# marl/l3embedding

Hardware: AMD Instinct MI355X
Metric: AVC training pairs/sec (1s audio + 224x224 frame) (higher is better)
Workload: dtype f32; 1 GPU; full cnn_L3_melspec2 AVC training step (audio+vision+fusion, fwd+bwd+Adam), batch 64 per GPU, global batch 64, fp32, inputs resident in HBM; global_batch=64, parallelism=dp1, fp32_conv=f4x4

## Files before the change

l3embedding_amd/csrc/conv_path.h:

```cpp
#pragma once
#include "kernels.h"

namespace l3 {

ConvGeom conv_geom(int n, int h, int w, int cin, int cout, int kh, int kw, bool same, int f2x2);
ConvGeom conv_dgrad_geom(const ConvGeom& g);

struct ConvStorage {
    bool mixed = false;
    bool x_bf16 = false, y_bf16 = false, dy_bf16 = false, dx_bf16 = false;
};

enum ConvFwd { CF_BF16_STORED, CF_BF16_CAST, CF_FIRST, CF_FP32 };
enum ConvWgrad { WG_BF16_STORED, WG_BF16_CAST, WG_FP32 };
enum ConvDgrad { DG_NONE, DG_SMALL, DG_BF16_STORED, DG_BF16_CAST, DG_WINO, DG_FLIPPED };
struct ConvFwdPath {
    ConvFwd path = CF_FP32;
    bool wino_filter = false;
    double executed = -1.0;
};
struct ConvWgradPath {
    ConvWgrad path = WG_FP32;
    double executed = -1.0;
};
struct ConvDgradPath {
    ConvDgrad path = DG_NONE;
    double executed = -1.0;
};
ConvFwdPath conv_resolve_fwd(const ConvGeom& g, const ConvStorage& st, bool have_u);
ConvWgradPath conv_resolve_wgrad(const ConvGeom& g, const ConvStorage& st);
ConvDgradPath conv_resolve_dgrad(const ConvGeom& g, const ConvGeom& dg, const ConvStorage& st, bool have_u);
int conv_fwd_stat_blocks(const ConvFwdPath& p, const ConvGeom& g);
int conv_dgrad_bn_blocks(const ConvDgradPath& p, const ConvGeom& dg, bool dx_bf16, bool bn_x_bf16);

struct ConvBufs {
    const float* x = nullptr;
    const float* w = nullptr;
    const float* bias = nullptr;
    float* y = nullptr;
    float* dx = nullptr;
    float* dw = nullptr;
    float* wprep = nullptr;
    float* wino_u = nullptr;
    bool u_ready = false;
    float* wg_part = nullptr;
    float* stat_part = nullptr;
    int stat_mode = 0;
    const BnBwdFuse* bn_bwd = nullptr;
};
void conv_run_fwd(const ConvFwdPath& p, const ConvGeom& g, const ConvStorage& st, const ConvBufs& b, hipStream_t s);
void conv_run_wgrad(const ConvWgradPath& p, const ConvGeom& g, const ConvBufs& b, hipStream_t s);
void conv_run_dgrad(const ConvDgradPath& p, const ConvGeom& g, const ConvGeom& dg, const ConvStorage& st, const ConvBufs& b, hipStream_t s);

}
```

l3embedding_amd/csrc/conv_path.hip:

```cpp
#include "conv_path.h"

namespace l3 {

ConvGeom conv_geom(int n, int h, int w, int cin, int cout, int kh, int kw, bool same, int f2x2) {
    ConvGeom g{n, h, w, cin, 0, 0, cout, kh, kw, 0, 0};
    if (same) {
        tf_same(h, kh, 1, &g.Ho, &g.padT);
        tf_same(w, kw, 1, &g.Wo, &g.padL);
    } else {
        g.Ho = h - kh + 1;
        g.Wo = w - kw + 1;
    }
    g.f2x2 = f2x2;
    return g;
}

ConvGeom conv_dgrad_geom(const ConvGeom& g) {
    ConvGeom dg{g.N, g.Ho, g.Wo, g.Cout, g.H, g.W, g.Cin, g.KH, g.KW, g.KH - 1 - g.padT, g.KW - 1 - g.padL};
    dg.f2x2 = g.f2x2;
    dg.solo = g.solo;
    return dg;
}

ConvFwdPath conv_resolve_fwd(const ConvGeom& g, const ConvStorage& st, bool have_u) {
    ConvFwdPath p;
    const bool mp = st.mixed && conv_bf16_ok(g);
    p.path = mp ? (st.x_bf16 ? CF_BF16_STORED : CF_BF16_CAST) : conv_first_ok(g) ? CF_FIRST : CF_FP32;
    p.wino_filter = have_u && !mp && conv_wino_ok(g);
    p.executed = p.wino_filter ? conv_wino_executed_flops(g) : -1.0;
    return p;
}

ConvWgradPath conv_resolve_wgrad(const ConvGeom& g, const ConvStorage& st) {
    ConvWgradPath p;
    const bool wbf = st.mixed && conv_wgrad_bf16_ok(g);
    p.path = !wbf ? WG_FP32 : st.x_bf16 && st.dy_bf16 ? WG_BF16_STORED : WG_BF16_CAST;
    p.executed = conv_wgrad_executed_flops(g, wbf);
    return p;
}

ConvDgradPath conv_resolve_dgrad(const ConvGeom& g, const ConvGeom& dg, const ConvStorage& st, bool have_u) {
    ConvDgradPath p;
    const bool dbf = st.mixed && conv_bf16_ok(dg), wino = have_u && conv_wino_ok(dg);
    p.path = conv_dgrad_small_ok(g) ? DG_SMALL : dbf ? (st.dy_bf16 ? DG_BF16_STORED : DG_BF16_CAST) : wino ? DG_WINO : DG_FLIPPED;
    p.executed = wino && !dbf ? conv_wino_executed_flops(dg) : -1.0;
    return p;
}

int conv_fwd_stat_blocks(const ConvFwdPath& p, const ConvGeom& g) {
    return p.path == CF_BF16_STORED ? conv_bf16_stat_blocks(g)
           : p.path == CF_FIRST     ? conv_first_stat_blocks(g)
           : p.path == CF_FP32 && p.wino_filter ? conv_wino_stat_blocks(g) : 0;
}

int conv_dgrad_bn_blocks(const ConvDgradPath& p, const ConvGeom& dg, bool dx_bf16, bool bn_x_bf16) {
    int blocks = -1;
    if (p.path == DG_BF16_STORED && dx_bf16 && bn_x_bf16 && conv_bf16_halo_ok(dg)) blocks = conv_bf16_stat_blocks(dg);
    if (p.path == DG_WINO && !dx_bf16 && !bn_x_bf16 && conv_wino_ok(dg)) blocks = conv_wino_stat_blocks(dg);
    return blocks;
}

void conv_run_fwd(const ConvFwdPath& p, const ConvGeom& g, const ConvStorage& st, const ConvBufs& b, hipStream_t s) {
    if (p.wino_filter && !b.u_ready) conv_wino_transform_weights(b.w, b.wino_u, g, false, s);
    switch (p.path) {
        case CF_BF16_STORED:
            conv_weights_bf16(b.w, b.wprep, g.KH, g.KW, g.Cin, g.Cout, true, s);
            conv_bf16_fwd(b.x, b.wprep, b.bias, b.y, g, s, true, b.stat_part, b.stat_mode, st.y_bf16);
            break;
        case CF_BF16_CAST:
            conv_flip_weights(b.w, b.wprep, g.KH, g.KW, g.Cin, g.Cout, s);
            conv_bf16_fwd(b.x, b.wprep, b.bias, b.y, g, s);
            break;
        case CF_FIRST:
            conv_first_fwd(b.x, b.w, b.bias, b.y, g, s, b.stat_part, b.stat_mode, st.y_bf16);
            break;
        case CF_FP32:
            conv_fwd(b.x, b.w, b.bias, b.y, g, s, p.wino_filter ? b.wino_u : nullptr, b.stat_part, b.stat_mode);
            break;
    }
}

void conv_run_wgrad(const ConvWgradPath& p, const ConvGeom& g, const ConvBufs& b, hipStream_t s) {
    conv_wgrad(b.x, b.y, b.dw, b.wg_part, g, s, p.path != WG_FP32, p.path == WG_BF16_STORED);
}

void conv_run_dgrad(const ConvDgradPath& p, const ConvGeom& g, const ConvGeom& dg, const ConvStorage& st, const ConvBufs& b, hipStream_t s) {
    switch (p.path) {
        case DG_SMALL:
            (void)conv_dgrad_small(b.y, b.w, b.dx, g, s);
            break;
        case DG_BF16_STORED:
            conv_weights_bf16(b.w, b.wprep, g.KH, g.KW, g.Cin, g.Cout, false, s);
            conv_bf16_fwd(b.y, b.wprep, nullptr, b.dx, dg, s, true, b.stat_part, 0, st.dx_bf16, b.bn_bwd);
            break;
        case DG_BF16_CAST:
            conv_bf16_fwd(b.y, b.w, nullptr, b.dx, dg, s);
            break;
        case DG_WINO:
            conv_wino_transform_weights(b.w, b.wino_u, dg, true, s);
            conv_fwd(b.y, nullptr, nullptr, b.dx, dg, s, b.wino_u, b.stat_part, 0, b.bn_bwd);
            break;
        case DG_FLIPPED:
            conv_flip_weights(b.w, b.wprep, g.KH, g.KW, g.Cin, g.Cout, s);
            conv_fwd(b.y, b.wprep, nullptr, b.dx, dg, s);
            break;
        case DG_NONE: break;
    }
}

}
```

l3embedding_amd/csrc/conv_wino4.hip:

```cpp
#include "kernels.h"
#include "device_common.h"

#include <stdlib.h>
#include <string.h>

#include <mutex>
#include <vector>

namespace l3 {

namespace {

struct Wino4Args {
    const float* x;
    const float* u;
    const float* bias;
    float* y;
    int N, H, W, Cin, Cout;
    int TY, TX;
    int tiles;
    int mblocks, nblocks, nchunks;
    float inv_tpi, inv_tx;
    float* stat_part;
    int stat_mode;
// ... 581 lines not shown
        if (t < 128) {
            const int c32 = t & 31, which = (t >> 5) & 1, jn = t >> 6;
            float sum = 0.f;
#pragma unroll
            for (int r = 0; r < NS; ++r) sum += red[((jn * 2 + which) * NS + r) * 32 + c32];
            a.stat_part[((size_t)mb * 2 + which) * a.Cout + n0 + jn * 32 + c32] = sum;
        }
    }
    if (!worker) __builtin_amdgcn_s_waitcnt(0x0070 | (0xF << 8));
    if (dyn && wave == 11 && lane0 == 0) {
        asm volatile("" ::: "memory");
        int nx = -1;
        if (has_next) {
            nx = wq_base(a.lt_first, xcd) + 8 * claim_k;
            if (nx >= a.lt_end) nx = wq_claim(a.work, xcd, 1, a.lt_first, a.lt_end);
        }
        Qw[it & 1] = nx;
    }
    have0 = has_next;
    }
    if (dyn && t == 0) wq_leave(a.work, (int)gridDim.x);
}

__global__ __launch_bounds__(256) void wino4_weights_kernel(const float* __restrict__ w, float* __restrict__ u, int Cin,
                                                            int Cout, int dgrad) {
    const int idx = blockIdx.x * 256 + threadIdx.x;
    if (idx >= Cin * Cout) return;
    const int k = idx % Cout, c = idx / Cout;
    float g[3][3];
#pragma unroll
    for (int kh = 0; kh < 3; ++kh)
#pragma unroll
        for (int kw = 0; kw < 3; ++kw)
            g[kh][kw] = dgrad ? w[((size_t)((2 - kh) * 3 + (2 - kw)) * Cout + k) * Cin + c]
                              : w[((size_t)(kh * 3 + kw) * Cin + c) * Cout + k];
    auto gmul = [](float a0, float a1, float a2, float* o) {
        const float s02 = a0 + a2;
        o[0] = a0;
        o[1] = (-1.f / 3.f) * (s02 + a1);
        o[2] = (1.f / 3.f) * (s02 - a1);
        o[3] = (1.f / 15.f) * fmaf(2.f, a1, fmaf(4.f, a2, a0));
        o[4] = (-4.f / 15.f) * fmaf(-2.f, a1, fmaf(4.f, a0, a2));
        o[5] = a2;
    };
    float gg[6][3];
#pragma unroll
    for (int kw = 0; kw < 3; ++kw) {
        float o[6];
        gmul(g[0][kw], g[1][kw], g[2][kw], o);
#pragma unroll
        for (int xi = 0; xi < 6; ++xi) gg[xi][kw] = o[xi];
    }
    const int c8 = c >> 3, hf = (c >> 2) & 1, sub = (c >> 1) & 1, c2 = c & 1;
#pragma unroll
    for (int xi = 0; xi < 6; ++xi) {
        float o[6];
        gmul(gg[xi][0], gg[xi][1], gg[xi][2], o);
#pragma unroll
        for (int nu = 0; nu < 6; ++nu)
            u[(((((size_t)(xi * 6 + nu) * (Cin >> 3) + c8) * 2 + sub) * 2 + hf) * Cout + k) * 2 + c2] = o[nu];
    }
}

template <int SM>
__global__ __launch_bounds__(256) void wino4_tail_reduce_kernel(Wino4Args a) {
    __shared__ float red[2][64][16];
    const int t = threadIdx.x, q = t & 3, slot = t >> 2;
    const int blk = (int)blockIdx.x >> 2, cg = (int)blockIdx.x & 3;
    const int lt = a.lt_first + blk;
    const int logical = xcd_remap(lt, a.mblocks * a.nblocks);
    const int nb = logical % a.nblocks, mb = logical / a.nblocks;
    const int n0 = nb * 64, T0 = mb * W4_TILES;
    const int cl = cg * 16 + 4 * q;
    const int ch = n0 + cl;
    f32x4 bz = {0.f, 0.f, 0.f, 0.f};
    if (a.bias != nullptr) bz = *reinterpret_cast<const f32x4*>(a.bias + ch);
    f32x4 bsc = bz, bsh = bz, bmu = bz, brs = bz;
    if constexpr (SM == 2) {
        bsc = *reinterpret_cast<const f32x4*>(a.bb.scale + ch);
        bsh = *reinterpret_cast<const f32x4*>(a.bb.shift + ch);
        bmu = *reinterpret_cast<const f32x4*>(a.bb.mean + ch);
        const f32x4 var = *reinterpret_cast<const f32x4*>(a.bb.var + ch);
#pragma unroll
        for (int c = 0; c < 4; ++c) brs[c] = rsqrtf(var[c] + a.bb.eps);
// ... 176 lines not shown
}

bool conv_wino4_selected(const ConvGeom& g) {
    const char* env = l3_knob("L3_WINO4");
    const int min_cin = env ? atoi(env) : 64;
    return !g.f2x2 && min_cin > 0 && g.Cin >= min_cin && g.Cin >= 16 && g.Cin % 8 == 0 && g.Cout % 64 == 0 &&
           (size_t)36 * g.Cin * g.Cout * 4 < (1ull << 31);
}

double conv_wino4_executed_flops(const ConvGeom& g) {
    return 2.0 * 36.0 * (double)g.N * ((g.H + 3) / 4) * ((g.W + 3) / 4) * (double)g.Cin * (double)g.Cout;
}

size_t conv_wino4_tail_scratch_bytes() { return (size_t)304 * W4_TILES * 16 * 64 * sizeof(float); }

int conv_wino4_blocks(const ConvGeom& g, int n) { return (n * ((g.H + 3) / 4) * ((g.W + 3) / 4) + W4_TILES - 1) / W4_TILES; }

void conv_wino4_transform_weights(const float* w, float* u, const ConvGeom& g, bool from_fwd_for_dgrad, hipStream_t s) {
    const int total = g.Cin * g.Cout;
    hipLaunchKernelGGL(wino4_weights_kernel, dim3((total + 255) / 256), dim3(256), 0, s, w, u, g.Cin, g.Cout,
                       from_fwd_for_dgrad ? 1 : 0);
}

void conv_wino4_launch(const float* x, const float* u, const float* bias, float* y, const ConvGeom& g, int n, hipStream_t s,
                       float* stat_part, int stat_mode, const BnBwdFuse* bn_bwd) {
    Wino4Args a;
    a.solo = g.solo;
    a.dynamic = g.dynamic;
    a.tail_buf = g.tail_scratch;
    a.tail_cap = g.tail_scratch_bytes;
    a.x = x; a.u = u; a.bias = bias; a.y = y;
    a.N = n; a.H = g.H; a.W = g.W; a.Cin = g.Cin; a.Cout = g.Cout;
    a.TY = (g.H + 3) / 4;
    a.TX = (g.W + 3) / 4;
    a.tiles = n * a.TY * a.TX;
    a.mblocks = conv_wino4_blocks(g, n);
    a.nblocks = g.Cout / 64;
    a.nchunks = g.Cin / 8;
    a.inv_tpi = 1.0f / (float)(a.TY * a.TX);
    a.inv_tx = 1.0f / (float)a.TX;
    a.stat_part = stat_part;
    a.stat_mode = stat_mode;
    a.bb = BnBwdFuse{nullptr, nullptr, nullptr, nullptr, nullptr, 0.f, 0};
    a.stagger_cycles = 0;
    a.stagger_groups = 1;
    a.lt_first = 0;
// ... 21 lines not shown
```

l3embedding_amd/csrc/engine.hip:

```cpp
#include <hip/hip_runtime.h>
#include "knobs.h"

#include <cmath>
#include <cstdio>
#include <cstdlib>
#include <cstring>
#include <map>
#include <string>
#include <vector>

#include "../../include/l3hip.h"
#include "comm.h"
#include "conv_path.h"
#include "featprep.h"
#include "kernels.h"

namespace {

using namespace l3;

static thread_local std::string g_create_error;

constexpr float BN_EPS = 1e-3f;
constexpr float BN_MOMENTUM = 0.99f;
// ... 18 lines not shown

struct Param {
    std::string name;
    int ndim = 0;
    int64_t shape[4] = {1, 1, 1, 1};
    bool trainable = false;
    int kind = 0;
    int64_t numel = 0;
    int bucket = 0;
    float* d = nullptr;
    float* g = nullptr;
};

enum FirstWgrad { FW_NONE, FW_AUG, FW_AUG_DEFERRED };
struct ConvPlan {
    ConvStorage st;
    ConvFwdPath fwd;
    int stat_mode = 0;
    FirstWgrad aug = FW_NONE;
    ConvWgradPath wgrad;
    bool colsum = false;
    ConvDgradPath dgrad;
    int bwd_bn = -1;
    double fwd_bytes = 0.0, wg_bytes = 0.0, dg_bytes = 0.0;
};
enum BnStats { BS_PARTIALS, BS_FAST, BS_PLAIN, BS_MOVING };
enum BnBwd { BB_BY_FIRST_CONV, BB_FAST_POOLED, BB_FAST, BB_FAST_DEFERRED, BB_PLAIN };
struct BnPlan {
    BnStats stats = BS_MOVING;
    int stat_blocks = 0;
    BnBwd bwd = BB_PLAIN;
    int bwd_blocks = 0;
    double fwd_bytes = 0.0, bwd_bytes = 0.0;
};

struct Op {
    OpKind kind;
    std::string name;
    int in = 0, out = 0;
    int block = 0, bucket = 0;
    int kh = 0, kw = 0, cout = 0;
    bool same = false;
    ConvGeom geom{};
    ConvGeom dgeom{};
    int p_kernel = -1, p_bias = -1;
    float* wflip = nullptr;
    float *wino_uf = nullptr, *wino_ud = nullptr;
    int in_bn = -1;
    bool fused_first = false;
    bool defer_apply = false;
    int bn_defer = -1;
    float *xaug = nullptr, *gaug = nullptr;
    ConvGeom ageom{};
    int bn_follow = -1;
    bool need_dx = true;
    int dy_to_bn = -1;
    float* xwin = nullptr;
    int p_gamma = -1, p_beta = -1, p_mmean = -1, p_mvar = -1;
    bool fused_relu = false;
    bool prerelu = false;
    int fuse_pool = -1;
    int bias_param = -1;
    bool fused_into_bn = false;
    bool bias_by_bn = false;
    float *mean = nullptr, *var = nullptr, *scale = nullptr, *shift = nullptr;
    float *biased_mean = nullptr, *biased_var = nullptr;
    PoolGeom pg{};
    ConvPlan cp{};
    BnPlan bp{};
};

struct Tower {
    std::string prefix;
    std::vector<Tensor> t;
    std::vector<Op> ops;
    int nblocks = 0;
    int emb_conv_op = -1;
    bool training = false;
};

struct FrontendDef {
    int n_dft, n_hop, same, n_mels, sqrt_out, db, loglambda;
    const char* layer_name;
};

struct ProfRec {
    int family;
    hipEvent_t a, b;
    double flops;
    double executed;
    double bytes;
    const char* tag;
};

}

struct l3_engine {
    l3_config cfg{};
    int B = 0;
    hipStream_t stream = nullptr;
    bool own_stream = false;
    hipStream_t side = nullptr;
    hipEvent_t ev_fork = nullptr, ev_join = nullptr;
    float *red_scratch2 = nullptr, *wg_scratch2 = nullptr;
    float *stat_scratch = nullptr, *stat_scratch2 = nullptr;
    size_t stat_max = 0;
    float* w4_tail = nullptr;
    bool overlap = true;
    BnMovingEntry* bn_table = nullptr;
    int bn_table_n = 0, bn_table_max_c = 0;
    std::string err;
    l3::DeviceBufs bufs;

    std::vector<Param> params;
    std::map<std::string, int> pindex;
    float *arena_p = nullptr, *arena_g = nullptr, *arena_m = nullptr, *arena_v = nullptr;
    int64_t n_train = 0;
    struct Segment { int64_t off, n; bool l2; };
    std::vector<Segment> segments;
    struct Bucket { int64_t off, n; };
    std::vector<Bucket> buckets;
    int64_t adam_t = 0;
    int64_t bn_step = 0;

    Tower vis, aud;
    FrontendDef fe{};
    FrontendCfg fcfg{};
    int p_real = -1, p_imag = -1, p_mel = -1;
    bool consts_dirty = true;
    float *wdft = nullptr, *melw = nullptr, *frames = nullptr, *spec = nullptr, *smax = nullptr;
    bool dft_consts_done = false;
    float *dft_win = nullptr, *dft_b1 = nullptr, *dft_b2 = nullptr, *dft_tw = nullptr, *dft_y = nullptr, *dft_a2 = nullptr, *dft_nyq = nullptr;
    int *mel_start = nullptr, *mel_len = nullptr, *mel_off = nullptr;
// ... 556 lines not shown
            memcpy(row, &real[(size_t)t * nb], nb * sizeof(float));
            memcpy(row + nb, &imag[(size_t)t * nb], nb * sizeof(float));
        }
        HIPCHK(e, hipMemcpy(e->wdft, w.data(), w.size() * 4, hipMemcpyHostToDevice));
    }
    if (f.n_mels) {
        std::vector<float> fb((size_t)nb * f.n_mels);
        HIPCHK(e, hipMemcpy(fb.data(), e->params[e->p_mel].d, fb.size() * 4, hipMemcpyDeviceToHost));
        MelBands bands;
        mel_pack_bands(fb.data(), nb, f.n_mels, bands);
        const std::vector<int>&st = bands.start, &ln = bands.len, &of = bands.off;
        const std::vector<float>& packed = bands.w;
        if ((int64_t)packed.size() > e->melw_cap) {
            e->err = "mel filterbank too dense for the band buffer";
            return L3_EINVAL;
        }
        HIPCHK(e, hipMemcpy(e->melw, packed.data(), packed.size() * 4, hipMemcpyHostToDevice));
        HIPCHK(e, hipMemcpy(e->mel_start, st.data(), st.size() * 4, hipMemcpyHostToDevice));
        HIPCHK(e, hipMemcpy(e->mel_len, ln.data(), ln.size() * 4, hipMemcpyHostToDevice));
        HIPCHK(e, hipMemcpy(e->mel_off, of.data(), of.size() * 4, hipMemcpyHostToDevice));
    }
    e->consts_dirty = false;
    return L3_OK;
}

int alloc_everything(l3_engine* e, uint64_t seed) {
    const int B = e->B;
    const int nbuckets = 1 + e->vis.nblocks + e->aud.nblocks;
    std::vector<int64_t> offs(e->params.size(), -1);
    int64_t off = 0;
    e->buckets.resize(nbuckets);
    for (int b = 0; b < nbuckets; ++b) {
        e->buckets[b].off = off;
        for (int pass = 0; pass < 2; ++pass) {
            const int64_t seg0 = off;
            for (size_t i = 0; i < e->params.size(); ++i) {
                Param& p = e->params[i];
                if (!p.trainable || p.bucket != b) continue;
                const bool is_l2 = p.kind == PK_KERNEL;
                if ((pass == 0) != is_l2) continue;
                offs[i] = off;
                off += (p.numel + 3) / 4 * 4;
            }
            if (off > seg0) e->segments.push_back({seg0, off - seg0, pass == 0});
        }
        e->buckets[b].n = off - e->buckets[b].off;
// ... 191 lines not shown
            }
        }
    }
    if (e->vis.ops.back().kind != OP_POOL || e->aud.ops.back().kind != OP_POOL) {
        e->err = "tower must end in a pooling layer";
        return L3_EINVAL;
    }
    if ((rc = dev_alloc_t(e, &e->red_scratch, red_max))) return rc;
    if ((rc = dev_alloc_t(e, &e->wg_scratch, wg_max))) return rc;
    if ((rc = dev_alloc_t(e, &e->sq_scratch, 2048))) return rc;
    if (stat_max && (rc = dev_alloc_t(e, &e->stat_scratch, stat_max))) return rc;
    {
        bool any_w4 = false;
        for (Tower* tw : {&e->vis, &e->aud})
            for (auto& op : tw->ops)
                if (op.kind == OP_CONV && (op.wino_uf || op.wino_ud)) any_w4 = true;
        if (any_w4 && e->cfg.dtype != L3_DTYPE_BF16 && (rc = dev_alloc_t(e, &e->w4_tail, conv_wino4_tail_scratch_bytes() / sizeof(float)))) return rc;
    }
    if (e->side) {
        if ((rc = dev_alloc_t(e, &e->red_scratch2, red_max))) return rc;
        if ((rc = dev_alloc_t(e, &e->wg_scratch2, wg_max))) return rc;
        if (stat_max && (rc = dev_alloc_t(e, &e->stat_scratch2, stat_max))) return rc;
    }
    return L3_OK;
}

int run_frontend(l3_engine* e) {
    int rc = rebuild_consts(e);
    if (rc) return rc;
    const FrontendCfg& f = e->fcfg;
    const int B = e->B;
    const int M = B * f.n_frames;
    const bool mag = e->cfg.frontend == L3_FRONTEND_MINISPEC && f.n_mels > 0;
    if (f.factored) {
        const int N1 = f.N1, N2 = f.N2;
        const int form = knob_int("L3_DFT_FACTORED", 1);
        if (form != 2 && f.n_mels > 0 && N1 == 32 && N2 == 64) {
            const double m1 = (double)M * N2, m2 = (double)M * N1;
            ProfScope ps(e, F_FRONTEND, 2.0 * M * (double)f.n_dft * 2.0 * f.n_freq + 2.0 * M * (double)f.n_freq * f.n_mels, nullptr,
                         2.0 * m1 * N1 * 2 * N1 + 2.0 * m2 * 2 * N2 * N2);
            dft_fused(e->audio, e->dft_win, e->dft_b1, e->dft_b2, e->dft_tw, e->melw, e->mel_start, e->mel_len, e->mel_off, e->aud.t[0].d, B,
                      AUDIO_T, f, e->stream, mag);
            if (f.db) db_normalize(e->aud.t[0].d, e->smax, B, e->aud.t[0].batch_stride, e->cfg.db_max_scope, e->stream);
            return L3_OK;
        }
        {
            ProfScope ps(e, F_FRONTEND, 0.0);
// ... 23 lines not shown
        {
            ProfScope ps(e, F_FRONTEND, 0.0);
            frame_audio(e->audio, e->frames, B, AUDIO_T, f, e->stream);
        }
        ConvGeom g{1, 1, M, f.n_dft, 1, M, f.ncols_pad, 1, 1, 0, 0};
        ProfScope ps(e, F_FRONTEND, 2.0 * M * (double)f.n_dft * 2.0 * f.n_freq);
        conv_fwd(e->frames, e->wdft, nullptr, e->spec, g, e->stream);
    }
    {
        ProfScope ps(e, F_FRONTEND, f.n_mels ? 2.0 * B * f.n_frames * (double)f.n_freq * f.n_mels : 0.0);
        spec_to_features(e->spec, e->melw, e->mel_start, e->mel_len, e->mel_off, e->aud.t[0].d, B, f, e->stream, e->dft_nyq, mag);
        if (f.db) db_normalize(e->aud.t[0].d, e->smax, B, e->aud.t[0].batch_stride, e->cfg.db_max_scope, e->stream);
    }
    return L3_OK;
}

static inline double act_bytes(const Tensor& t) { return (double)t.numel() * (t.d_bf16 ? 2.0 : 4.0); }
static inline double grad_bytes(const Tensor& t) { return (double)t.numel() * (t.g_bf16 ? 2.0 : 4.0); }

int plan_tower(l3_engine* e, Tower& tw, bool training, int solo) {
    static const int epi_stats = knob_int("L3_EPILOGUE_STATS", 1);
    const bool bf16 = e->cfg.dtype == L3_DTYPE_BF16;
    tw.training = training;
    auto fits = [&](const Op& cv, int blocks, int C) {
        if ((size_t)blocks * 2 * C <= e->stat_max) return true;
        e->err = cv.name + ": " + std::to_string(blocks) + " partial blocks of " + std::to_string(C) + " channels exceed the statistics scratch (" +
                 std::to_string(e->stat_max) + " floats)";
        return false;
    };
    auto defers = [&](const Op& bn) {
        return training && bn.defer_apply && bn.fuse_pool < 0 && bn_fast_ok(tw.t[bn.in].C) && tw.t[bn.in].d_bf16 == tw.t[bn.out].g_bf16;
    };
    for (auto& op : tw.ops) op.bp = BnPlan{};
    for (auto& op : tw.ops) {
        if (op.kind != OP_CONV) continue;
        op.geom.solo = op.dgeom.solo = solo;
        op.geom.dynamic = op.dgeom.dynamic = e->comm != nullptr ? 1 : 0;
        float* ts = solo ? e->w4_tail : nullptr;
        op.geom.tail_scratch = op.dgeom.tail_scratch = ts;
        op.geom.tail_scratch_bytes = op.dgeom.tail_scratch_bytes = ts ? conv_wino4_tail_scratch_bytes() : 0;

        const Tensor &x = tw.t[op.in], &y = tw.t[op.out];
        const double wbytes = (double)e->params[op.p_kernel].numel * 4.0;
        ConvPlan& p = op.cp = ConvPlan{};
        p.st = ConvStorage{bf16, x.d_bf16, y.d_bf16, y.g_bf16, x.g_bf16};
        p.fwd = conv_resolve_fwd(op.geom, p.st, op.wino_uf != nullptr);
        p.fwd_bytes = act_bytes(x) + act_bytes(y) + wbytes;
        const int nblk = conv_fwd_stat_blocks(p.fwd, op.geom);
        if (epi_stats && training && op.bn_follow >= 0 && e->stat_max > 0 && nblk > 0) {
            if (!fits(op, nblk, op.geom.Cout)) return L3_ESTATE;
            p.stat_mode = tw.ops[op.bn_follow].prerelu ? 2 : 1;
            tw.ops[op.bn_follow].bp.stat_blocks = nblk;
        }
        if (training && op.in_bn >= 0) {
            const Op* fb = op.bn_defer >= 0 && defers(tw.ops[op.bn_defer]) ? &tw.ops[op.bn_defer] : nullptr;
            p.aug = fb ? FW_AUG_DEFERRED : FW_AUG;
            p.wg_bytes = (double)x.rows() * op.ageom.Cin * 4.0 + (fb ? act_bytes(tw.t[fb->in]) + grad_bytes(tw.t[fb->out]) : grad_bytes(y));
            continue;
        }
        p.wgrad = conv_resolve_wgrad(op.geom, p.st);
        p.wg_bytes = act_bytes(x) + grad_bytes(y) + wbytes;
        p.colsum = !op.bias_by_bn;
        if (!op.need_dx) continue;
        p.dgrad = conv_resolve_dgrad(op.geom, op.dgeom, p.st, op.wino_ud != nullptr);
        p.dg_bytes = grad_bytes(y) + grad_bytes(x) + wbytes;
        Op* bn = training && op.dy_to_bn >= 0 && e->stat_max > 0 ? &tw.ops[op.dy_to_bn] : nullptr;
        if (bn != nullptr && bn->fuse_pool >= 0 && (bn->xwin == nullptr || x.batch_stride != (int64_t)x.H * x.W * x.C)) bn = nullptr;
        if (bn == nullptr) continue;
        const int blocks = conv_dgrad_bn_blocks(p.dgrad, op.dgeom, x.g_bf16, tw.t[bn->in].d_bf16);
        if (blocks < 0) continue;
        if (!fits(op, blocks, op.dgeom.Cout)) return L3_ESTATE;
        p.bwd_bn = op.dy_to_bn;
        bn->bp.bwd_blocks = blocks;
    }
    for (auto& op : tw.ops) {
        if (op.kind != OP_BN) continue;
        const Tensor &x = tw.t[op.in], &y = tw.t[op.out];
        const Tensor& out = op.fuse_pool >= 0 ? tw.t[tw.ops[op.fuse_pool].out] : y;
        BnPlan& p = op.bp;
        p.stats = !training ? BS_MOVING : p.stat_blocks > 0 ? BS_PARTIALS : op.prerelu || x.d_bf16 ? BS_FAST : BS_PLAIN;
        p.bwd = training && op.fused_first ? BB_BY_FIRST_CONV : !bn_fast_ok(x.C) ? BB_PLAIN : op.fuse_pool >= 0 ? BB_FAST_POOLED
                : defers(op) ? BB_FAST_DEFERRED : BB_FAST;
        p.fwd_bytes = (!training ? 0.0 : p.stat_blocks > 0 ? (double)p.stat_blocks * 2 * x.C * 4 : act_bytes(x)) + act_bytes(x) + act_bytes(out);
        if (p.bwd == BB_BY_FIRST_CONV) p.fwd_bytes += act_bytes(x) + (double)x.rows() * (&op + 1)->ageom.Cin * 4.0;
        if (op.fuse_pool >= 0 && training && op.xwin != nullptr) p.fwd_bytes += (double)out.numel() * (x.d_bf16 ? 2.0 : 4.0);
        p.bwd_bytes = p.bwd == BB_PLAIN ? 2.0 * (act_bytes(x) + grad_bytes(y)) + grad_bytes(x)
                                        : (p.bwd_blocks > 0 ? (double)p.bwd_blocks * 2 * x.C * 4 : act_bytes(x) + grad_bytes(out)) +
                                              (p.bwd == BB_FAST_DEFERRED ? 0.0 : act_bytes(x) + grad_bytes(out) + grad_bytes(x));
    }
    return L3_OK;
}

void tower_forward(l3_engine* e, Tower& tw) {
    const bool training = tw.training;
    for (auto& op : tw.ops) {
        Tensor& x = tw.t[op.in];
        Tensor& y = tw.t[op.out];
        switch (op.kind) {
            case OP_CONV: {
                const ConvPlan& p = op.cp;
                ConvBufs b;
                b.x = x.d, b.w = e->params[op.p_kernel].d, b.bias = e->params[op.p_bias].d, b.y = y.d;
                b.wprep = op.wflip, b.wino_u = op.wino_uf;
                b.stat_part = p.stat_mode ? e->stat_scratch : nullptr, b.stat_mode = p.stat_mode;
                ProfScope ps(e, F_CONV_FWD, conv_flops(op.geom), op.name.c_str(), p.fwd.executed);
                ps.bytes(p.fwd_bytes);
                conv_run_fwd(p.fwd, op.geom, p.st, b, e->stream);
                break;
            }
            case OP_BN: {
                const BnPlan& p = op.bp;
                ProfScope ps(e, F_ELEMWISE, 0.0);
                ps.bytes(p.fwd_bytes);
                const float* gamma = e->params[op.p_gamma].d;
                const float* beta = e->params[op.p_beta].d;
                switch (p.stats) {
                    case BS_PARTIALS:
                        bn_stats_from_partials(e->stat_scratch, p.stat_blocks, e->params[op.bias_param].d, gamma, beta, op.mean, op.var,
                                               op.scale, op.shift, x.rows(), x.C, BN_EPS, op.prerelu ? 1 : 0, e->stream);
                        break;
                    case BS_FAST:
                        bn_stats_fast(x.d, gamma, beta, op.mean, op.var, op.scale, op.shift, e->red_scratch, x.rows(), x.C, BN_EPS,
                                      op.prerelu ? 1 : 0, e->stream, x.d_bf16 ? 1 : 0);
                        break;
                    case BS_PLAIN:
                        bn_stats(x.d, gamma, beta, op.mean, op.var, op.scale, op.shift, e->red_scratch, x.rows(), x.C, BN_EPS, e->stream);
// ... 91 lines not shown
                if (p.aug != FW_NONE) {
                    ProfScope ps(e, F_CONV_WGRAD, conv_flops(op.geom), op.name.c_str());
                    ps.bytes(p.wg_bytes);
                    const Op& bn = tw.ops[op.in_bn];
                    if (p.aug == FW_AUG_DEFERRED) {
                        const Op& fb = tw.ops[op.bn_defer];
                        const Tensor &bi = tw.t[fb.in], &bo = tw.t[fb.out];
                        const float* co = bn_bwd_fast_coeffs(e->red_scratch, op.cout);
                        const FirstWgFuse f{bi.d, bo.g, fb.scale, fb.shift, co, co + op.cout, co + 2 * op.cout, fb.fused_relu ? 1 : 0,
                                            bi.d_bf16 ? 1 : 0};
                        conv_wgrad(op.xaug, nullptr, op.gaug, e->wg_scratch, op.ageom, e->stream, false, false, &f);
                    } else {
                        conv_wgrad(op.xaug, y.g, op.gaug, e->wg_scratch, op.ageom, e->stream);
                    }
                    first_conv_grads(op.gaug, w, e->params[bn.p_gamma].d, e->params[bn.p_beta].d, e->params[op.p_kernel].g,
                                     e->params[bn.p_gamma].g, e->params[bn.p_beta].g,
                                     op.bias_by_bn && p.aug == FW_AUG ? nullptr : e->params[op.p_bias].g, op.kh * op.kw, x.C, op.cout,
                                     e->stream);
                    break;
                }
                ConvBufs b;
                b.x = x.d, b.w = w, b.y = y.g, b.dx = x.g, b.dw = e->params[op.p_kernel].g;
                b.wprep = op.wflip, b.wino_u = op.wino_ud, b.wg_part = e->wg_scratch;
                {
                    ProfScope ps(e, F_CONV_WGRAD, conv_flops(op.geom), op.name.c_str(), p.wgrad.executed);
                    ps.bytes(p.wg_bytes);
                    conv_run_wgrad(p.wgrad, op.geom, b, e->stream);
                }
                if (p.colsum) {
                    ProfScope ps(e, F_ELEMWISE, 0.0);
                    ps.bytes(grad_bytes(y));
                    colsum(y.g, e->params[op.p_bias].g, e->red_scratch, y.rows(), y.C, e->stream);
                }
                if (p.dgrad.path == DG_NONE) break;
                ProfScope ps(e, F_CONV_DGRAD, conv_flops(op.geom), op.name.c_str(), p.dgrad.executed);
                ps.bytes(p.dg_bytes);
                BnBwdFuse bb{};
                if (p.bwd_bn >= 0) {
                    bb = bn_bwd_fuse(tw, tw.ops[p.bwd_bn]);
                    b.bn_bwd = &bb, b.stat_part = e->stat_scratch;
                }
                conv_run_dgrad(p.dgrad, op.geom, op.dgeom, p.st, b, e->stream);
                break;
            }
            default: break;
        }
// ... 107 lines not shown
    e->bn_table_n = (int)tab.size();
    e->bn_pack_floats = off;
    BnMovingEntry* dev = nullptr;
    if (int rc = dev_alloc_t(e, &dev, tab.size() + 1)) return rc;
    HIPCHK(e, hipMemcpy(dev, tab.data(), tab.size() * sizeof(BnMovingEntry), hipMemcpyHostToDevice));
    e->bn_table = dev;
    return L3_OK;
}

int bn_stats_pack(l3_engine* e, int world, int slot = -1) {
    int rc = ensure_bn_table(e);
    if (rc) return rc;
    if (e->bn_pack_floats == 0) return L3_OK;
    if (slot < 0 && e->bn_send == nullptr && (rc = dev_alloc_t(e, &e->bn_send, (size_t)e->bn_pack_floats))) return rc;
    if (e->bn_gathered_world < world) {
        if ((rc = dev_alloc_t(e, &e->bn_gathered, (size_t)e->bn_pack_floats * world))) return rc;
        e->bn_gathered_world = world;
    }
    bn_moving_pack(e->bn_table, e->bn_table_n, e->bn_table_max_c,
                   slot < 0 ? e->bn_send : e->bn_gathered + (size_t)slot * e->bn_pack_floats, e->stream);
    return L3_OK;
}

int do_update(l3_engine* e, float lr, float grad_scale) {
    {
        ProfScope ps(e, F_ADAM, 0.0);
        e->adam_t += 1;
        const double t = (double)e->adam_t;
        const float lr_t = lr * (sqrtf(1.f - powf(ADAM_B2, (float)t)) / (1.f - powf(ADAM_B1, (float)t)));
        for (size_t i = 0; i < e->segments.size(); ++i) {
            const auto& s = e->segments[i];
            int64_t n = s.n;
            const int64_t n_l2 = s.l2 ? s.n : 0;
            if (s.l2 && i + 1 < e->segments.size() && !e->segments[i + 1].l2 && e->segments[i + 1].off == s.off + s.n)
                n += e->segments[++i].n;
            adam_step(e->arena_p + s.off, e->arena_g + s.off, e->arena_m + s.off, e->arena_v + s.off, n, n_l2, 2.f * L2_WEIGHT,
                      lr_t, ADAM_B1, ADAM_B2, ADAM_EPS, grad_scale, e->stream);
        }
    }
    ProfScope ps(e, F_ELEMWISE, 0.0);
    int rc = ensure_bn_table(e);
    if (rc) return rc;
    const int replicas = e->bn_replicas_armed;
    e->bn_replicas_armed = 0;
    e->bn_step += replicas > 0 ? replicas : 1;
    bn_moving_update_all(e->bn_table, e->bn_table_n, e->bn_table_max_c, BN_MOMENTUM, e->cfg.bn_zero_debias, e->bn_step, e->stream,
                         replicas > 0 ? e->bn_gathered : nullptr, replicas, e->bn_pack_floats);
    return L3_OK;
}

int read_results(l3_engine* e, float* loss, float* acc, float* probs, float* logits) {
    HIPCHK(e, l3::stream_wait(e->stream));
    prof_collect(e);
    float st[16], l2[64];
    HIPCHK(e, hipMemcpy(st, e->stats, sizeof(st), hipMemcpyDeviceToHost));
    HIPCHK(e, hipMemcpy(l2, e->l2part, sizeof(l2), hipMemcpyDeviceToHost));
    double reg = 0.0;
    int si = 0;
    for (auto& s : e->segments)
        if (s.l2) reg += (double)L2_WEIGHT * (double)l2[si++];
// ... 238 lines not shown
    auto it = e->pindex.find(name);
    if (it == e->pindex.end()) {
        e->err = std::string("unknown parameter: ") + name;
        return L3_EINVAL;
    }
    Param& p = e->params[it->second];
    if (p.numel != numel) {
        e->err = std::string("size mismatch for ") + name + ": expected " + std::to_string(p.numel) + " got " +
                 std::to_string(numel);
        return L3_EINVAL;
    }
    *out = &p;
    return L3_OK;
}

int l3_set_param(l3_engine* e, const char* name, const float* src, int64_t numel) {
    Param* p;
    int rc = find_param(e, name, numel, &p);
    if (rc) return rc;
    HIPCHK(e, hipSetDevice(e->cfg.device));
    HIPCHK(e, l3::stream_wait(e->stream));
    HIPCHK(e, hipMemcpy(p->d, src, (size_t)numel * 4, hipMemcpyHostToDevice));
    if (p->kind == PK_CONST) e->consts_dirty = true;
    return L3_OK;
}

int l3_get_param(l3_engine* e, const char* name, float* dst, int64_t numel) {
    Param* p;
    int rc = find_param(e, name, numel, &p);
    if (rc) return rc;
    HIPCHK(e, hipSetDevice(e->cfg.device));
    HIPCHK(e, l3::stream_wait(e->stream));
    HIPCHK(e, hipMemcpy(dst, p->d, (size_t)numel * 4, hipMemcpyDeviceToHost));
    return L3_OK;
}

int l3_get_grad(l3_engine* e, const char* name, float* dst, int64_t numel) {
    Param* p;
    int rc = find_param(e, name, numel, &p);
    if (rc) return rc;
    if (!p->trainable) {
        e->err = std::string("not trainable: ") + name;
        return L3_EINVAL;
    }
    HIPCHK(e, hipSetDevice(e->cfg.device));
    HIPCHK(e, l3::stream_wait(e->stream));
// ... 33 lines not shown
    const size_t nb = (size_t)src->n_train * 4;
    HIPCHK(dst, hipMemcpyAsync(dst->arena_p, src->arena_p, nb, hipMemcpyDeviceToDevice, dst->stream));
    HIPCHK(dst, hipMemcpyAsync(dst->arena_m, src->arena_m, nb, hipMemcpyDeviceToDevice, dst->stream));
    HIPCHK(dst, hipMemcpyAsync(dst->arena_v, src->arena_v, nb, hipMemcpyDeviceToDevice, dst->stream));
    for (size_t i = 0; i < src->params.size(); ++i) {
        const Param& ps = src->params[i];
        if (ps.trainable) continue;
        HIPCHK(dst, hipMemcpyAsync(dst->params[i].d, ps.d, (size_t)ps.numel * 4, hipMemcpyDeviceToDevice, dst->stream));
    }
    Tower* dt[2] = {&dst->vis, &dst->aud};
    Tower* st[2] = {&src->vis, &src->aud};
    for (int t = 0; t < 2; ++t)
        for (size_t i = 0; i < st[t]->ops.size(); ++i) {
            const Op& so = st[t]->ops[i];
            Op& dop = dt[t]->ops[i];
            if (so.kind != OP_BN) continue;
            const size_t n = (size_t)(st[t]->t[so.in].C + 3) / 4 * 4 * 4;
            HIPCHK(dst, hipMemcpyAsync(dop.biased_mean, so.biased_mean, n, hipMemcpyDeviceToDevice, dst->stream));
            HIPCHK(dst, hipMemcpyAsync(dop.biased_var, so.biased_var, n, hipMemcpyDeviceToDevice, dst->stream));
        }
    dst->adam_t = src->adam_t;
    dst->bn_step = src->bn_step;
    dst->consts_dirty = true;
    HIPCHK(dst, l3::stream_wait(dst->stream));
    return L3_OK;
}

int l3_optimizer_steps(const l3_engine* e, int64_t* adam_t, int64_t* bn_steps) {
    if (!e) return L3_EINVAL;
    if (adam_t) *adam_t = e->adam_t;
    if (bn_steps) *bn_steps = e->bn_step;
    return L3_OK;
}

int l3_upload_batch(l3_engine* e, const float* video, const float* audio, const float* labels) {
    if (!e) return L3_EINVAL;
    HIPCHK(e, hipSetDevice(e->cfg.device));
    return upload_inputs(e, video, audio, labels);
}

int l3_upload_batch_raw(l3_engine* e, const uint8_t* video_u8, const int16_t* audio_i16, const int32_t* labels_i32) {
    if (!e) return L3_EINVAL;
    HIPCHK(e, hipSetDevice(e->cfg.device));
    return e->feed.upload(BATCH_SINGLE, 1, video_u8, audio_i16, labels_i32, nullptr, nullptr, e->stream, &e->err);
}

// ... 1488 lines not shown
```

l3embedding_amd/csrc/kernels.h:

```cpp
#pragma once
#include <hip/hip_runtime.h>
#include <stdint.h>

#include <string>
#include <vector>

#include "host_common.h"

struct l3_clipbank;
struct l3_sample;

namespace l3 {

struct ConvGeom {
    int N, H, W, Cin;
    int Ho, Wo, Cout;
    int KH, KW, padT, padL;
    int f2x2 = 0;
    int solo = 0;
    int dynamic = 0;
    float* tail_scratch = nullptr;
    size_t tail_scratch_bytes = 0;
};
size_t conv_wino4_tail_scratch_bytes();

struct BnBwdFuse {
    const float* x;
    const float *scale, *shift;
    const float *mean, *var;
    float eps;
    int relu;
};
void conv_fwd(const float* x, const float* w, const float* bias, float* y, const ConvGeom& g,
              hipStream_t s, const float* wino_u = nullptr, float* bn_part = nullptr, int bn_mode = 0,
              const BnBwdFuse* bn_bwd = nullptr);
bool conv_wino_ok(const ConvGeom& g);
size_t conv_wino_floats(const ConvGeom& g);
double conv_wino_executed_flops(const ConvGeom& g);
void conv_wino_transform_weights(const float* w, float* u, const ConvGeom& g, bool from_fwd_for_dgrad, hipStream_t s);
void conv_wino_fwd(const float* x, const float* u, const float* bias, float* y, const ConvGeom& g, hipStream_t s,
                   float* stat_part = nullptr, int stat_mode = 0, const BnBwdFuse* bn_bwd = nullptr);
int conv_wino_stat_blocks(const ConvGeom& g);
int conv_wino_stat_blocks_max(const ConvGeom& g);
bool conv_dgrad_small_ok(const ConvGeom& g);
bool conv_dgrad_small(const float* dy, const float* w, float* dx, const ConvGeom& g, hipStream_t s);
void conv_flip_weights(const float* w, float* wt, int KH, int KW, int Cin, int Cout, hipStream_t s);
size_t conv_wgrad_scratch_floats(const ConvGeom& g);
bool conv_wgrad_bf16_ok(const ConvGeom& g);
struct FirstWgFuse;
void conv_wgrad(const float* x, const float* dy, float* dw, float* part, const ConvGeom& g,
                hipStream_t s, bool bf16 = false, bool in_bf16 = false, const FirstWgFuse* first_fuse = nullptr);

bool conv_first_ok(const ConvGeom& g);
bool conv_first_wgrad_ok(const ConvGeom& g);
size_t conv_first_wgrad_scratch_floats(const ConvGeom& g);
struct FirstWgFuse {
    const void *bnx, *dA;
    const float *scale, *shift;
    const float *cA, *cB, *cC;
    int relu;
    int bf16;
};
int conv_first_wgrad(const float* x, const float* dy, float* part, const ConvGeom& g, hipStream_t s, const FirstWgFuse* fuse = nullptr);
int conv_first_stat_blocks(const ConvGeom& g);
// ... 285 lines not shown
```

Baseline: 2069 pairs/s.

## Cache Winograd F(4x4) filter transforms and rebuild them in batched launch after Adam

Keeps transformed Winograd weights valid across forward and dgrad calls. They are invalidated only when kernels change. After each Adam segment update, all affected F(4x4) filters of a bucket are regenerated in one table-driven batched kernel launch. This replaces the per-conv transform launches in the forward and backward passes. It adds validity-flag bookkeeping, and it risks stale filters if a weight-mutating path misses invalidation.

```diff
diff --git a/l3embedding_amd/csrc/conv_path.h b/l3embedding_amd/csrc/conv_path.h
--- a/l3embedding_amd/csrc/conv_path.h
+++ b/l3embedding_amd/csrc/conv_path.h
@@ -17,6 +17,7 @@
 struct ConvFwdPath {
     ConvFwd path = CF_FP32;
     bool wino_filter = false;
+    bool u_f4x4 = false;
     double executed = -1.0;
 };
 struct ConvWgradPath {
@@ -25,6 +26,7 @@
 };
 struct ConvDgradPath {
     ConvDgrad path = DG_NONE;
+    bool u_f4x4 = false;
     double executed = -1.0;
 };
 ConvFwdPath conv_resolve_fwd(const ConvGeom& g, const ConvStorage& st, bool have_u);
@@ -43,6 +45,7 @@
     float* wprep = nullptr;
     float* wino_u = nullptr;
     bool u_ready = false;
+    bool* u_valid = nullptr;
     float* wg_part = nullptr;
     float* stat_part = nullptr;
     int stat_mode = 0;
diff --git a/l3embedding_amd/csrc/conv_path.hip b/l3embedding_amd/csrc/conv_path.hip
--- a/l3embedding_amd/csrc/conv_path.hip
+++ b/l3embedding_amd/csrc/conv_path.hip
@@ -27,6 +27,7 @@
     const bool mp = st.mixed && conv_bf16_ok(g);
     p.path = mp ? (st.x_bf16 ? CF_BF16_STORED : CF_BF16_CAST) : conv_first_ok(g) ? CF_FIRST : CF_FP32;
     p.wino_filter = have_u && !mp && conv_wino_ok(g);
+    p.u_f4x4 = p.wino_filter && conv_wino4_selected(g);
     p.executed = p.wino_filter ? conv_wino_executed_flops(g) : -1.0;
     return p;
 }
@@ -43,6 +44,7 @@
     ConvDgradPath p;
     const bool dbf = st.mixed && conv_bf16_ok(dg), wino = have_u && conv_wino_ok(dg);
     p.path = conv_dgrad_small_ok(g) ? DG_SMALL : dbf ? (st.dy_bf16 ? DG_BF16_STORED : DG_BF16_CAST) : wino ? DG_WINO : DG_FLIPPED;
+    p.u_f4x4 = p.path == DG_WINO && conv_wino4_selected(dg);
     p.executed = wino && !dbf ? conv_wino_executed_flops(dg) : -1.0;
     return p;
 }
@@ -60,8 +62,14 @@
     return blocks;
 }
 
+static void wino_filter(const ConvBufs& b, const ConvGeom& g, bool from_fwd_for_dgrad, hipStream_t s) {
+    if (b.u_ready || (b.u_valid != nullptr && *b.u_valid)) return;
+    conv_wino_transform_weights(b.w, b.wino_u, g, from_fwd_for_dgrad, s);
+    if (b.u_valid != nullptr) *b.u_valid = true;
+}
+
 void conv_run_fwd(const ConvFwdPath& p, const ConvGeom& g, const ConvStorage& st, const ConvBufs& b, hipStream_t s) {
-    if (p.wino_filter && !b.u_ready) conv_wino_transform_weights(b.w, b.wino_u, g, false, s);
+    if (p.wino_filter) wino_filter(b, g, false, s);
     switch (p.path) {
         case CF_BF16_STORED:
             conv_weights_bf16(b.w, b.wprep, g.KH, g.KW, g.Cin, g.Cout, true, s);
@@ -97,7 +105,7 @@
             conv_bf16_fwd(b.y, b.w, nullptr, b.dx, dg, s);
             break;
         case DG_WINO:
-            conv_wino_transform_weights(b.w, b.wino_u, dg, true, s);
+            wino_filter(b, dg, true, s);
             conv_fwd(b.y, nullptr, nullptr, b.dx, dg, s, b.wino_u, b.stat_part, 0, b.bn_bwd);
             break;
         case DG_FLIPPED:
diff --git a/l3embedding_amd/csrc/conv_wino4.hip b/l3embedding_amd/csrc/conv_wino4.hip
--- a/l3embedding_amd/csrc/conv_wino4.hip
+++ b/l3embedding_amd/csrc/conv_wino4.hip
@@ -627,10 +627,8 @@
     if (dyn && t == 0) wq_leave(a.work, (int)gridDim.x);
 }
 
-__global__ __launch_bounds__(256) void wino4_weights_kernel(const float* __restrict__ w, float* __restrict__ u, int Cin,
-                                                            int Cout, int dgrad) {
-    const int idx = blockIdx.x * 256 + threadIdx.x;
-    if (idx >= Cin * Cout) return;
+__device__ __forceinline__ void wino4_weights_one(const float* __restrict__ w, float* __restrict__ u, int Cin, int Cout, int dgrad,
+                                                  int idx) {
     const int k = idx % Cout, c = idx / Cout;
     float g[3][3];
 #pragma unroll
@@ -665,6 +663,18 @@
         for (int nu = 0; nu < 6; ++nu)
             u[(((((size_t)(xi * 6 + nu) * (Cin >> 3) + c8) * 2 + sub) * 2 + hf) * Cout + k) * 2 + c2] = o[nu];
     }
+}
+__global__ __launch_bounds__(256) void wino4_weights_kernel(const float* __restrict__ w, float* __restrict__ u, int Cin,
+                                                            int Cout, int dgrad) {
+    const int idx = blockIdx.x * 256 + threadIdx.x;
+    if (idx >= Cin * Cout) return;
+    wino4_weights_one(w, u, Cin, Cout, dgrad, idx);
+}
+__global__ __launch_bounds__(256) void wino4_weights_table_kernel(const Wino4FilterEntry* __restrict__ tab) {
+    const Wino4FilterEntry en = tab[blockIdx.y];
+    const int idx = blockIdx.x * 256 + threadIdx.x;
+    if (idx >= en.Cin * en.Cout) return;
+    wino4_weights_one(en.w, en.u, en.Cin, en.Cout, en.dgrad, idx);
 }
 
 template <int SM>
@@ -887,6 +897,11 @@
                        from_fwd_for_dgrad ? 1 : 0);
 }
 
+void conv_wino4_transform_weights_table(const Wino4FilterEntry* tab_dev, int entries, int max_pairs, hipStream_t s) {
+    if (entries <= 0 || max_pairs <= 0) return;
+    hipLaunchKernelGGL(wino4_weights_table_kernel, dim3((max_pairs + 255) / 256, entries), dim3(256), 0, s, tab_dev);
+}
+
 void conv_wino4_launch(const float* x, const float* u, const float* bias, float* y, const ConvGeom& g, int n, hipStream_t s,
                        float* stat_part, int stat_mode, const BnBwdFuse* bn_bwd) {
     Wino4Args a;
diff --git a/l3embedding_amd/csrc/engine.hip b/l3embedding_amd/csrc/engine.hip
--- a/l3embedding_amd/csrc/engine.hip
+++ b/l3embedding_amd/csrc/engine.hip
@@ -64,6 +64,7 @@
     bool colsum = false;
     ConvDgradPath dgrad;
     int bwd_bn = -1;
+    bool keep_uf = false, keep_ud = false;
     double fwd_bytes = 0.0, wg_bytes = 0.0, dg_bytes = 0.0;
 };
 enum BnStats { BS_PARTIALS, BS_FAST, BS_PLAIN, BS_MOVING };
@@ -88,6 +89,7 @@
     int p_kernel = -1, p_bias = -1;
     float* wflip = nullptr;
     float *wino_uf = nullptr, *wino_ud = nullptr;
+    bool uf_valid = false, ud_valid = false;
     int in_bn = -1;
     bool fused_first = false;
     bool defer_apply = false;
@@ -119,6 +121,7 @@
     int nblocks = 0;
     int emb_conv_op = -1;
     bool training = false;
+    bool u_cache = true;
 };
 
 struct FrontendDef {
@@ -151,6 +154,11 @@
     bool overlap = true;
     BnMovingEntry* bn_table = nullptr;
     int bn_table_n = 0, bn_table_max_c = 0;
+    Wino4FilterEntry* u_table = nullptr;
+    struct FilterRef { int tower, op, dgrad; };
+    std::vector<FilterRef> u_refs;
+    struct FilterRange { int first = 0, count = 0, max_pairs = 0; };
+    std::vector<FilterRange> u_buckets;
     std::string err;
     l3::DeviceBufs bufs;
 
@@ -753,6 +761,46 @@
     }
     e->consts_dirty = false;
     return L3_OK;
+}
+
+int build_filter_table(l3_engine* e) {
+    std::vector<Wino4FilterEntry> tab;
+    e->u_buckets.assign(e->buckets.size(), l3_engine::FilterRange{});
+    for (int b = 0; b < (int)e->buckets.size(); ++b) {
+        l3_engine::FilterRange& r = e->u_buckets[b];
+        r.first = (int)tab.size();
+        for (int ti = 0; ti < 2; ++ti) {
+            Tower& tw = ti == 0 ? e->vis : e->aud;
+            for (int oi = 0; oi < (int)tw.ops.size(); ++oi) {
+                const Op& op = tw.ops[oi];
+                if (op.kind != OP_CONV || op.bucket != b) continue;
+                const Tensor &x = tw.t[op.in], &y = tw.t[op.out];
+                const ConvStorage st{e->cfg.dtype == L3_DTYPE_BF16, x.d_bf16, y.d_bf16, y.g_bf16, x.g_bf16};
+                const float* w = e->params[op.p_kernel].d;
+                if (conv_resolve_fwd(op.geom, st, op.wino_uf != nullptr).u_f4x4) {
+                    tab.push_back(Wino4FilterEntry{w, op.wino_uf, op.geom.Cin, op.geom.Cout, 0});
+                    e->u_refs.push_back({ti, oi, 0});
+                    r.max_pairs = std::max(r.max_pairs, op.geom.Cin * op.geom.Cout);
+                }
+                if (op.in_bn < 0 && op.need_dx && conv_resolve_dgrad(op.geom, op.dgeom, st, op.wino_ud != nullptr).u_f4x4) {
+                    tab.push_back(Wino4FilterEntry{w, op.wino_ud, op.dgeom.Cin, op.dgeom.Cout, 1});
+                    e->u_refs.push_back({ti, oi, 1});
+                    r.max_pairs = std::max(r.max_pairs, op.dgeom.Cin * op.dgeom.Cout);
+                }
+            }
+        }
+        r.count = (int)tab.size() - r.first;
+    }
+    if (tab.empty()) return L3_OK;
+    if (int rc = dev_alloc_t(e, &e->u_table, tab.size())) return rc;
+    HIPCHK(e, hipMemcpy(e->u_table, tab.data(), tab.size() * sizeof(Wino4FilterEntry), hipMemcpyHostToDevice));
+    return L3_OK;
+}
+
+void filters_invalidate(l3_engine* e, int pi = -1) {
+    for (Tower* tw : {&e->vis, &e->aud})
+        for (auto& op : tw->ops)
+            if (op.kind == OP_CONV && (pi < 0 || op.p_kernel == pi)) op.uf_valid = op.ud_valid = false;
 }
 
 int alloc_everything(l3_engine* e, uint64_t seed) {
@@ -990,7 +1038,7 @@
         if ((rc = dev_alloc_t(e, &e->wg_scratch2, wg_max))) return rc;
         if (stat_max && (rc = dev_alloc_t(e, &e->stat_scratch2, stat_max))) return rc;
     }
-    return L3_OK;
+    return build_filter_table(e);
 }
 
 int run_frontend(l3_engine* e) {
@@ -1060,6 +1108,7 @@
     static const int epi_stats = knob_int("L3_EPILOGUE_STATS", 1);
     const bool bf16 = e->cfg.dtype == L3_DTYPE_BF16;
     tw.training = training;
+    tw.u_cache = knob_int("L3_U_CACHE", 1) != 0;
     auto fits = [&](const Op& cv, int blocks, int C) {
         if ((size_t)blocks * 2 * C <= e->stat_max) return true;
         e->err = cv.name + ": " + std::to_string(blocks) + " partial blocks of " + std::to_string(C) + " channels exceed the statistics scratch (" +
@@ -1083,6 +1132,7 @@
         ConvPlan& p = op.cp = ConvPlan{};
         p.st = ConvStorage{bf16, x.d_bf16, y.d_bf16, y.g_bf16, x.g_bf16};
         p.fwd = conv_resolve_fwd(op.geom, p.st, op.wino_uf != nullptr);
+        p.keep_uf = tw.u_cache && p.fwd.u_f4x4;
         p.fwd_bytes = act_bytes(x) + act_bytes(y) + wbytes;
         const int nblk = conv_fwd_stat_blocks(p.fwd, op.geom);
         if (epi_stats && training && op.bn_follow >= 0 && e->stat_max > 0 && nblk > 0) {
@@ -1101,6 +1151,7 @@
         p.colsum = !op.bias_by_bn;
         if (!op.need_dx) continue;
         p.dgrad = conv_resolve_dgrad(op.geom, op.dgeom, p.st, op.wino_ud != nullptr);
+        p.keep_ud = tw.u_cache && p.dgrad.u_f4x4;
         p.dg_bytes = grad_bytes(y) + grad_bytes(x) + wbytes;
         Op* bn = training && op.dy_to_bn >= 0 && e->stat_max > 0 ? &tw.ops[op.dy_to_bn] : nullptr;
         if (bn != nullptr && bn->fuse_pool >= 0 && (bn->xwin == nullptr || x.batch_stride != (int64_t)x.H * x.W * x.C)) bn = nullptr;
@@ -1140,6 +1191,8 @@
                 ConvBufs b;
                 b.x = x.d, b.w = e->params[op.p_kernel].d, b.bias = e->params[op.p_bias].d, b.y = y.d;
                 b.wprep = op.wflip, b.wino_u = op.wino_uf;
+                if (!p.keep_uf) op.uf_valid = false;
+                b.u_valid = p.keep_uf ? &op.uf_valid : nullptr;
                 b.stat_part = p.stat_mode ? e->stat_scratch : nullptr, b.stat_mode = p.stat_mode;
                 ProfScope ps(e, F_CONV_FWD, conv_flops(op.geom), op.name.c_str(), p.fwd.executed);
                 ps.bytes(p.fwd_bytes);
@@ -1277,6 +1330,8 @@
                 ConvBufs b;
                 b.x = x.d, b.w = w, b.y = y.g, b.dx = x.g, b.dw = e->params[op.p_kernel].g;
                 b.wprep = op.wflip, b.wino_u = op.wino_ud, b.wg_part = e->wg_scratch;
+                if (!p.keep_ud) op.ud_valid = false;
+                b.u_valid = p.keep_ud ? &op.ud_valid : nullptr;
                 {
                     ProfScope ps(e, F_CONV_WGRAD, conv_flops(op.geom), op.name.c_str(), p.wgrad.executed);
                     ps.bytes(p.wg_bytes);
@@ -1430,6 +1485,22 @@
     return L3_OK;
 }
 
+void filters_rebuild(l3_engine* e, int bucket) {
+    for (Tower* tw : {&e->vis, &e->aud})
+        for (auto& op : tw->ops)
+            if (op.kind == OP_CONV && op.bucket == bucket) op.uf_valid = op.ud_valid = false;
+    const l3_engine::FilterRange& r = e->u_buckets[bucket];
+    if (r.count == 0) return;
+    for (int i = r.first; i < r.first + r.count; ++i)
+        if (!(e->u_refs[i].tower == 0 ? e->vis : e->aud).u_cache) return;
+    conv_wino4_transform_weights_table(e->u_table + r.first, r.count, r.max_pairs, e->stream);
+    for (int i = r.first; i < r.first + r.count; ++i) {
+        const l3_engine::FilterRef& f = e->u_refs[i];
+        Op& op = (f.tower == 0 ? e->vis : e->aud).ops[f.op];
+        (f.dgrad ? op.ud_valid : op.uf_valid) = true;
+    }
+}
+
 int do_update(l3_engine* e, float lr, float grad_scale) {
     {
         ProfScope ps(e, F_ADAM, 0.0);
@@ -1444,6 +1515,8 @@
                 n += e->segments[++i].n;
             adam_step(e->arena_p + s.off, e->arena_g + s.off, e->arena_m + s.off, e->arena_v + s.off, n, n_l2, 2.f * L2_WEIGHT,
                       lr_t, ADAM_B1, ADAM_B2, ADAM_EPS, grad_scale, e->stream);
+            for (int b = 0; b < (int)e->buckets.size(); ++b)
+                if (e->buckets[b].off >= s.off && e->buckets[b].off + e->buckets[b].n <= s.off + n) filters_rebuild(e, b);
         }
     }
     ProfScope ps(e, F_ELEMWISE, 0.0);
@@ -1728,6 +1801,7 @@
     HIPCHK(e, l3::stream_wait(e->stream));
     HIPCHK(e, hipMemcpy(p->d, src, (size_t)numel * 4, hipMemcpyHostToDevice));
     if (p->kind == PK_CONST) e->consts_dirty = true;
+    if (p->kind == PK_KERNEL) filters_invalidate(e, (int)(p - e->params.data()));
     return L3_OK;
 }
 
@@ -1807,6 +1881,7 @@
     dst->adam_t = src->adam_t;
     dst->bn_step = src->bn_step;
     dst->consts_dirty = true;
+    filters_invalidate(dst);
     HIPCHK(dst, l3::stream_wait(dst->stream));
     return L3_OK;
 }
diff --git a/l3embedding_amd/csrc/kernels.h b/l3embedding_amd/csrc/kernels.h
--- a/l3embedding_amd/csrc/kernels.h
+++ b/l3embedding_amd/csrc/kernels.h
@@ -40,6 +40,13 @@
 void conv_wino_transform_weights(const float* w, float* u, const ConvGeom& g, bool from_fwd_for_dgrad, hipStream_t s);
 void conv_wino_fwd(const float* x, const float* u, const float* bias, float* y, const ConvGeom& g, hipStream_t s,
                    float* stat_part = nullptr, int stat_mode = 0, const BnBwdFuse* bn_bwd = nullptr);
+bool conv_wino4_selected(const ConvGeom& g);
+struct Wino4FilterEntry {
+    const float* w;
+    float* u;
+    int Cin, Cout, dgrad;
+};
+void conv_wino4_transform_weights_table(const Wino4FilterEntry* tab_dev, int entries, int max_pairs, hipStream_t s);
 int conv_wino_stat_blocks(const ConvGeom& g);
 int conv_wino_stat_blocks_max(const ConvGeom& g);
 bool conv_dgrad_small_ok(const ConvGeom& g);
```

After: 2065 pairs/s. No clear change (-0.2%).
